# dusk-network/dusk-blindbidproof

Hardware: AMD Instinct MI355X
Metric: blind-bid proofs/sec (higher is better)
Workload: dtype u32

## Files before the change

dusk_blindbidproof_amd/csrc/msm.hip:

```cpp
#include "context.h"

namespace bbp {

#ifndef BBP_FOLD_PRIO
#define BBP_FOLD_PRIO 2
#endif
#ifndef BBP_MSM_WAVES
#define BBP_MSM_WAVES 2
#endif
#ifndef BBP_MSM_WAVES_MAX
#define BBP_MSM_WAVES_MAX 2
#endif

#ifdef BBP_MSM_PROF
__device__ unsigned long long g_msm_prof[8];
#define MSM_PROF_BEGIN() unsigned long long prof_t = wall_clock64()
#define MSM_PROF_MARK(i)                                                    \
    if (tid == 0) {                                                         \
        unsigned long long now_ = wall_clock64();                           \
        atomicAdd(&g_msm_prof[i], now_ - prof_t);                           \
        prof_t = now_;                                                      \
    }
#else
#define MSM_PROF_BEGIN()
#define MSM_PROF_MARK(i)
#endif

__device__ __forceinline__ ge ge_shfl_down(const ge& p, int d) {
    ge r;
    const u32* w = reinterpret_cast<const u32*>(&p);
    u32* o = reinterpret_cast<u32*>(&r);
#pragma unroll
    for (int i = 0; i < GE_WORDS; i++) o[i] = (u32)__shfl_down((int)w[i], d, 64);
    return r;
}

__device__ __forceinline__ void xch_put(u32* xch, const ge& p) {
    const u32* w = reinterpret_cast<const u32*>(&p);
#pragma unroll
    for (int i = 0; i < GE_WORDS; i++) xch[i] = w[i];
}

__device__ __forceinline__ ge xch_get(const u32* xch) {
    ge p;
    u32* w = reinterpret_cast<u32*>(&p);
#pragma unroll
    for (int i = 0; i < GE_WORDS; i++) w[i] = xch[i];
    return p;
}

__device__ __forceinline__ row_regs load_row(const niels_row* __restrict__ tab, u32 entry, u32* __restrict__ fault) {
    u32 row = entry & 0x7fffffffu;
    if (row > (u32)(TAB_BASES * MSM_POS - 1)) {
        row = (u32)(TAB_BASES * MSM_POS - 1);
        atomicOr(fault, 1u);
    }
#ifdef BBP_EXP_ROWMASK
    row &= BBP_EXP_ROWMASK;
#endif
    return load_row_at(tab + row, entry >> 31);
}

#ifdef BBP_ACC_COOP
constexpr int COOP_IMG = 64 * 128;
__device__ __forceinline__ u32 coop_clamp_row(u32 entry, u32* __restrict__ fault) {
    u32 row = entry & 0x7fffffffu;
    if (row > (u32)(TAB_BASES * MSM_POS - 1)) {
        row = (u32)(TAB_BASES * MSM_POS - 1);
        atomicOr(fault, 1u);
    }
    return row;
}
__device__ __forceinline__ void coop_issue(const niels_row* __restrict__ tab, u8* wb, u32 my_row, int lane, u32 srcoff) {
    const u8* t = reinterpret_cast<const u8*>(tab);
    u32 r[8];
#pragma unroll
    for (int j = 0; j < 8; j++) r[j] = (u32)__shfl((int)my_row, 8 * j + (lane >> 3), 64);
#pragma unroll
    for (int j = 0; j < 8; j++) {
        const u8* src = t + (size_t)r[j] * 128 + (srcoff ^ (u32)((j & 1) << 6));
        __builtin_amdgcn_global_load_lds((const __attribute__((address_space(1))) void*)src, (__attribute__((address_space(3))) void*)(wb + j * 1024), 16, 0, 0);
    }
}
__device__ __forceinline__ row_regs coop_read(const u8* wb, u32 A, u32 neg) {
    const u32 An = A ^ (neg << 6);
    const uint4 a0 = *reinterpret_cast<const uint4*>(wb + An), a1 = *reinterpret_cast<const uint4*>(wb + (An ^ 0x10u));
    const uint2 a2 = *reinterpret_cast<const uint2*>(wb + (An ^ 0x20u));
    const uint4 b0 = *reinterpret_cast<const uint4*>(wb + (An ^ 0x40u)), b1 = *reinterpret_cast<const uint4*>(wb + (An ^ 0x50u));
    const uint2 b2 = *reinterpret_cast<const uint2*>(wb + (An ^ 0x60u));
    const uint2 x0 = *reinterpret_cast<const uint2*>(wb + (A ^ 0x20u) + 8);
    const uint4 x1 = *reinterpret_cast<const uint4*>(wb + (A ^ 0x30u));
    const uint2 x2 = *reinterpret_cast<const uint2*>(wb + (A ^ 0x60u) + 8), x3 = *reinterpret_cast<const uint2*>(wb + (A ^ 0x70u));
    row_regs r;
    r.ypx = fe{{(i32)a0.x, (i32)a0.y, (i32)a0.z, (i32)a0.w, (i32)a1.x, (i32)a1.y, (i32)a1.z, (i32)a1.w, (i32)a2.x, (i32)a2.y}};
    r.ymx = fe{{(i32)b0.x, (i32)b0.y, (i32)b0.z, (i32)b0.w, (i32)b1.x, (i32)b1.y, (i32)b1.z, (i32)b1.w, (i32)b2.x, (i32)b2.y}};
    r.xy2d = fe{{(i32)x0.x, (i32)x0.y, (i32)x1.x, (i32)x1.y, (i32)x1.z, (i32)x1.w, (i32)x2.x, (i32)x2.y, (i32)x3.x, (i32)x3.y}};
    return r;
}
#endif

__device__ __noinline__ void ge_add_nc(ge& r, const ge& a, const ge& b) { r = ge_add(a, b); }
__device__ __noinline__ void ge_dbl_nc(ge& r, const ge& a) { r = ge_dbl(a); }

#ifndef BBP_SORT_T
#define BBP_SORT_T 1024
#endif
constexpr int SORT_T = BBP_SORT_T;
template <int MODE> struct msm_geom;
template <> struct msm_geom<0> { static constexpr int K = MSM_K, NAF = MSM_NAF, W = MSM_W; };
template <> struct msm_geom<1> { static constexpr int K = FOLD_K, NAF = FOLD_NAF, W = FOLD_W; };
template <> struct msm_geom<2> { static constexpr int K = SMALL_K, NAF = SMALL_NAF, W = SMALL_W; };

template <int MODE>
__global__ __launch_bounds__(SORT_T) void k_msm_sort(const u32* __restrict__ scal_a, const u32* __restrict__ aux, u32 n_total, u32 n_idx_sets,
                                                      u32 n_sub, u32 split, u32* __restrict__ sorted_all, u32* __restrict__ cursor_all,
                                                      const u32* __restrict__ msm_map, const u32* __restrict__ n_active, u32* __restrict__ ticket) {
    constexpr int K = msm_geom<MODE>::K, NAF = msm_geom<MODE>::NAF, W = msm_geom<MODE>::W, G = K >= SORT_T ? K / SORT_T : 1;
    __shared__ u32 cursor[K + 1];
    __shared__ u32 part[SORT_T];
    const int tid = threadIdx.x;
    if (ticket && blockIdx.x == 0 && tid == 0) *ticket = 0;
    if (n_active && blockIdx.x >= *n_active) return;
    const size_t work = blockIdx.x, msm = work / split;
    const u32 i0 = (u32)(work % split) * n_sub;
    const u32 n = i0 < n_total ? min(n_sub, n_total - i0) : 0u;
    __builtin_amdgcn_s_setprio(3);
    const u32* sbase;
    const u32* base_idx = nullptr;
    u32 base0 = 0;
    if (MODE != 1) {
        const size_t src = msm_map ? (size_t)msm_map[msm] : msm;
        sbase = scal_a + (src * (size_t)n_total + i0) * 8;
        base_idx = aux + (size_t)(msm % n_idx_sets) * n_total + i0;
    } else {
        const u32 side = (u32)msm & 1u;
        sbase = (side ? aux : scal_a) + ((msm >> 1) * (size_t)2048 + i0) * 8;
        base0 = (side ? BBP_BASE_H0 : BBP_BASE_G0) + i0;
    }
    u32* sorted = sorted_all + work * (size_t)n_sub * W;
    auto key = [&](u32 i, u32 mag) -> u32 { return (MODE != 1 ? 0u : ((i0 + i) & (FOLD_CLS - 1)) * FOLD_M) + ((mag + 1) >> 1); };

    for (int k = tid; k <= K; k += SORT_T) cursor[k] = 0;
    __syncthreads();
    for (u32 i = tid; i < n; i += SORT_T) {
        const uint4* sp = reinterpret_cast<const uint4*>(sbase + (size_t)i * 8);
        uint4 lo = sp[0], hi = sp[1];
        const u32 s[8] = {lo.x, lo.y, lo.z, lo.w, hi.x, hi.y, hi.z, hi.w};
        if (MODE != 1 && base_idx[i] == MSM_SKIP_BASE) continue;
        sc_for_each_naf_digit<NAF>(s, [&](u32, u32 mag, u32) { atomicAdd(&cursor[key(i, mag)], 1u); });
    }
    __syncthreads();
    {
        u32 local = 0;
        for (int r = 1; r <= G; r++)
            if (tid * G + r <= K) local += cursor[tid * G + r];
        const int lane = tid & 63, wave = tid >> 6;
        u32 incl = local;
#pragma unroll
        for (int d = 1; d < 64; d <<= 1) {
            const u32 up = (u32)__shfl_up((int)incl, d, 64);
            if (lane >= d) incl += up;
        }
        if (lane == 63) part[wave] = incl;
        __syncthreads();
        if (tid < 64) {
            constexpr int NW = SORT_T / 64;
            u32 v = tid < NW ? part[tid] : 0u, sc_ = v;
#pragma unroll
            for (int d = 1; d < 64; d <<= 1) {
                const u32 up = (u32)__shfl_up((int)sc_, d, 64);
                if (tid >= d) sc_ += up;
            }
            if (tid < NW) part[tid] = sc_ - v;
        }
        __syncthreads();
        u32 base = part[wave] + incl - local;
        for (int r = 1; r <= G; r++) {
            if (tid * G + r > K) break;
            const u32 c = cursor[tid * G + r];
            cursor[tid * G + r] = base;
            base += c;
        }
    }
    __syncthreads();
    for (u32 i = tid; i < n; i += SORT_T) {
        const uint4* sp = reinterpret_cast<const uint4*>(sbase + (size_t)i * 8);
        uint4 lo = sp[0], hi = sp[1];
        const u32 s[8] = {lo.x, lo.y, lo.z, lo.w, hi.x, hi.y, hi.z, hi.w};
        if (MODE != 1 && base_idx[i] == MSM_SKIP_BASE) continue;
        const u32 tb = (MODE != 1 ? base_idx[i] : base0 + i) * MSM_POS;
        sc_for_each_naf_digit<NAF>(s, [&](u32 pos, u32 mag, u32 neg) {
            u32 at = atomicAdd(&cursor[key(i, mag)], 1u);
            sorted[at] = (tb + pos) | (neg << 31);
        });
    }
    __syncthreads();
    u32* cur_out = cursor_all + work * (size_t)(K + 1);
    for (int k = tid; k <= K; k += SORT_T) cur_out[k] = k ? cursor[k] : 0u;
}

template <int MODE> struct sort_cap { static constexpr u32 V = BBP_SORT_CAP; };
#ifndef BBP_SORT_CAP_FOLD
#define BBP_SORT_CAP_FOLD 8192
#endif
template <> struct sort_cap<1> { static constexpr u32 V = BBP_SORT_CAP_FOLD; };
constexpr int SORT_S = 3, SORT_S_WIDE = 5, SORT_S_FOLD = 2;
constexpr int SORT_MAXW = 62;
static_assert((u32)SORT_S_WIDE * SORT_T >= SORT_STAGED_MAX_TERMS && SORT_S_FOLD * SORT_T >= 2048 && SORT_MAXW + 2 <= SORT_T, "staged sort geometry");

#ifdef BBP_MSM_PROF
__device__ unsigned long long g_sort_prof[4][16];
#define SORT_PROF_MARK(i)                                                   \
    if (tid == 0) {                                                         \
        unsigned long long now_ = wall_clock64();                           \
        atomicAdd(&g_sort_prof[prof_cls][(i) < 15 ? (i) : 14], now_ - prof_t); \
        prof_t = now_;                                                      \
    }
#else
#define SORT_PROF_MARK(i)
#endif

template <int MODE, int S>
__global__ __launch_bounds__(SORT_T) void k_msm_sort_staged(const u32* __restrict__ scal_a, const u32* __restrict__ aux, u32 n_total, u32 n_idx_sets,
                                                             u32 n_sub, u32 split, u32* __restrict__ sorted_all, u32* __restrict__ cursor_all,
                                                             const u32* __restrict__ msm_map, const u32* __restrict__ n_active, u32 CAP, u32* __restrict__ ticket) {
    constexpr int K = msm_geom<MODE>::K, NAF = msm_geom<MODE>::NAF, W = msm_geom<MODE>::W, G = K >= SORT_T ? K / SORT_T : 1;
    constexpr int P = naf_slots<NAF>::P, NSLOT = naf_slots<NAF>::N, DW = naf_slots<NAF>::WORDS;
    extern __shared__ u32 stage[];
    __shared__ u32 start[K + 2];
    __shared__ u32 fill[K + 1];
    __shared__ u32 part[SORT_T];
    const int tid = threadIdx.x;
    if (ticket && blockIdx.x == 0 && tid == 0) *ticket = 0;
    if (n_active && blockIdx.x >= *n_active) return;
    const size_t work = blockIdx.x, msm = work / split;
    const u32 i0 = (u32)(work % split) * n_sub;
    const u32 n = i0 < n_total ? min(n_sub, n_total - i0) : 0u;
    __builtin_amdgcn_s_setprio(3);
    const u32* sbase;
    const u32* base_idx = nullptr;
    u32 base0 = 0;
    if (MODE != 1) {
        const size_t src = msm_map ? (size_t)msm_map[msm] : msm;
        sbase = scal_a + (src * (size_t)n_total + i0) * 8;
        base_idx = aux + (size_t)(msm % n_idx_sets) * n_total + i0;
    } else {
        const u32 side = (u32)msm & 1u;
        sbase = (side ? aux : scal_a) + ((msm >> 1) * (size_t)2048 + i0) * 8;
        base0 = (side ? BBP_BASE_H0 : BBP_BASE_G0) + i0;
    }
    u32* sorted = sorted_all + work * (size_t)n_sub * W;
    auto key = [&](u32 i, u32 mag) -> u32 { return (MODE != 1 ? 0u : ((i0 + i) & (FOLD_CLS - 1)) * FOLD_M) + ((mag + 1) >> 1); };

#ifdef BBP_MSM_PROF
    const int prof_cls = MODE == 1 ? 3 : n_sub <= 2049 ? 0 : n_sub <= SORT_WIDE_FROM ? 1 : 2;
    if (tid == 0) atomicAdd(&g_sort_prof[prof_cls][15], 1ull);
    unsigned long long prof_t = wall_clock64();
#endif
    for (int k = tid; k <= K; k += SORT_T) fill[k] = 0;
    __syncthreads();
    u32 dig[S][DW], valid[S], tb[S], koff[S];
#pragma unroll
    for (int j = 0; j < S; j++) {
        const u32 i = (u32)tid + (u32)j * SORT_T;
        valid[j] = 0, tb[j] = 0, koff[j] = 0;
#pragma unroll
        for (int d = 0; d < DW; d++) dig[j][d] = 0;
        if (i < n) {
            const uint4* sp = reinterpret_cast<const uint4*>(sbase + (size_t)i * 8);
            uint4 lo = sp[0], hi = sp[1];
            const u32 s[8] = {lo.x, lo.y, lo.z, lo.w, hi.x, hi.y, hi.z, hi.w};
            const u32 b = MODE != 1 ? base_idx[i] : base0 + i;
            if (MODE == 1 || b != MSM_SKIP_BASE) {
                tb[j] = b * MSM_POS;
                koff[j] = key(i, 0);
                const u32 ko = koff[j];
                sc_naf_digits_packed<NAF>(s, dig[j], valid[j], [&](u32 p) { atomicAdd(&fill[ko + naf_packed_bucket(p)], 1u); });
            }
        }
    }
    __syncthreads();
    SORT_PROF_MARK(0);
    {
        u32 local = 0;
        for (int r = 1; r <= G; r++)
            if (tid * G + r <= K) local += fill[tid * G + r];
        const int lane = tid & 63, wave = tid >> 6;
        u32 incl = local;
#pragma unroll
        for (int d = 1; d < 64; d <<= 1) {
            const u32 up = (u32)__shfl_up((int)incl, d, 64);
            if (lane >= d) incl += up;
        }
        if (lane == 63) part[wave] = incl;
        __syncthreads();
        if (tid < 64) {
            constexpr int NW = SORT_T / 64;
            u32 v = tid < NW ? part[tid] : 0u, sc_ = v;
#pragma unroll
            for (int d = 1; d < 64; d <<= 1) {
                const u32 up = (u32)__shfl_up((int)sc_, d, 64);
                if (tid >= d) sc_ += up;
            }
            if (tid < NW) part[tid] = sc_ - v;
        }
        __syncthreads();
        u32 base = part[wave] + incl - local;
        for (int r = 1; r <= G; r++) {
            if (tid * G + r > K) break;
            const u32 c = fill[tid * G + r];
            start[tid * G + r] = base;
            fill[tid * G + r] = 0;
            base += c;
        }
        if (tid == SORT_T - 1) start[K + 1] = base;
        if (tid == 0) start[0] = 0;
    }
    __syncthreads();
    u32 kb0 = 1;
    while (kb0 <= (u32)K) {
        if (tid < 64) {
            u32 kb = kb0, nw = 0;
            while (kb <= (u32)K && nw < (u32)SORT_MAXW) {
                const u32 base = start[kb];
                u32 ke = kb + 1;
                if (start[ke] - base <= CAP) {
                    u32 lo = kb + 1, hi = (u32)K + 1;
                    while (lo < hi) {
                        const u32 mid = (lo + hi + 1) >> 1;
                        if (start[mid] - base <= CAP) lo = mid; else hi = mid - 1;
                    }
                    ke = lo;
                }
                if (start[ke] != base) {
                    if (tid == 0) part[1 + nw] = ke;
                    nw++;
                }
                kb = ke;
            }
            if (tid == 0) part[0] = nw, part[1 + nw] = kb;
        }
        __syncthreads();
        SORT_PROF_MARK(2);
        const u32 nw = (u32)__builtin_amdgcn_readfirstlane((int)part[0]);
        u32 kb = kb0;
        for (u32 w = 0; w < nw; w++) {
            const u32 ke = (u32)__builtin_amdgcn_readfirstlane((int)part[1 + w]);
            const u32 base = (u32)__builtin_amdgcn_readfirstlane((int)start[kb]), cnt = (u32)__builtin_amdgcn_readfirstlane((int)start[ke]) - base;
            const bool direct = cnt > CAP;
#pragma unroll
            for (int j = 0; j < S; j++) {
                asm volatile("" : "+v"(valid[j]));
#pragma unroll
                for (int d = 0; d < DW; d++) asm volatile("" : "+v"(dig[j][d]));
                if (!valid[j]) continue;
#pragma unroll
                for (int t = 0; t < NSLOT; t++) {
                    if (!(valid[j] >> t & 1)) continue;
                    const u32 p = naf_slot<NAF>(dig[j], t), k = koff[j] + naf_packed_bucket(p);
                    if (k - kb < ke - kb) {
                        const u32 at = start[k] + atomicAdd(&fill[k], 1u);
                        const u32 ent = (tb[j] + naf_packed_pos(p, t / P)) | (naf_packed_neg(p) << 31);
                        if (direct) sorted[at] = ent; else stage[at - base] = ent;
                    }
                }
            }
            __syncthreads();
            SORT_PROF_MARK(3 + 2 * w);
            if (!direct) {
                for (u32 i = tid; i < cnt; i += SORT_T) sorted[base + i] = stage[i];
                __syncthreads();
            }
            SORT_PROF_MARK(4 + 2 * w);
            kb = ke;
        }
        kb0 = (u32)__builtin_amdgcn_readfirstlane((int)part[1 + nw]);
        __syncthreads();
    }
    u32* cur_out = cursor_all + work * (size_t)(K + 1);
    for (int k = tid; k <= K; k += SORT_T) cur_out[k] = k ? start[k + 1] : 0u;
}

#ifndef BBP_ACC_WG
#define BBP_ACC_WG 256
#endif
constexpr int ACC_WG = BBP_ACC_WG, ACC_WGS = ACC_T / ACC_WG;
static_assert(ACC_T % ACC_WG == 0 && ACC_WG % 64 == 0, "accumulate workgroup geometry");

template <int MODE>
__global__ __launch_bounds__(ACC_WG) __attribute__((amdgpu_waves_per_eu(BBP_MSM_WAVES, BBP_MSM_WAVES_MAX)))
void k_msm_acc(const niels_row* __restrict__ ptable, const u32* __restrict__ sorted_all, const u32* __restrict__ cursor_all, u32 n ,
               ge* __restrict__ bsum_all, ge* __restrict__ psum_all, ge* __restrict__ out, const u32* __restrict__ n_active, u32* __restrict__ fault,
               u32 n_work, u32* __restrict__ ticket) {
    constexpr int K = msm_geom<MODE>::K, W = msm_geom<MODE>::W, G = K / MSM_T;
    __shared__ u32 cursor[K + 1];
#ifdef BBP_ACC_PERSIST
    static_assert(ACC_WGS == 1, "the persistent form draws whole MSMs");
    __shared__ u32 s_ticket;
  for (;;) {
    __syncthreads();
    if (threadIdx.x == 0) s_ticket = atomicAdd(ticket, 1u);
    __syncthreads();
    const size_t msm = s_ticket;
    if (msm >= n_work || (n_active && msm >= *n_active)) return;
    const int tid = (int)threadIdx.x;
#else
    const size_t msm = blockIdx.x / ACC_WGS;
    const int tid = (int)(blockIdx.x % ACC_WGS) * ACC_WG + (int)threadIdx.x;
    if (n_active && msm >= *n_active) return;
#endif
    const u32* sorted = sorted_all + msm * (size_t)n * W;
#ifdef BBP_MSM_PRIO
    __builtin_amdgcn_s_setprio(BBP_MSM_PRIO);
#endif
    MSM_PROF_BEGIN();
    {
        const u32* cur_in = cursor_all + msm * (size_t)(K + 1);
        for (int k = threadIdx.x; k <= K; k += ACC_WG) cursor[k] = cur_in[k];
    }
    __syncthreads();
    MSM_PROF_MARK(1);

    const u32 E = cursor[K];
    ge* bsum = bsum_all + msm * (size_t)K;
    ge* psum = psum_all + msm * (size_t)ACC_T;
#ifdef BBP_KO_ACC_PERMILLE
    const u32 c0 = (u32)(((u64)tid * E) / ACC_T), c1 = c0 + (u32)(((u64)((u32)(((u64)(tid + 1) * E) / ACC_T) - c0) * BBP_KO_ACC_PERMILLE) / 1000);
#else
    const u32 c0 = (u32)(((u64)tid * E) / ACC_T), c1 = (u32)(((u64)(tid + 1) * E) / ACC_T);
#endif
#ifdef BBP_MSM_PROF
    const unsigned long long clk0 = clock64();
#endif
    u32 k_first = 0;
    bool inside = false;
#ifdef BBP_ACC_COOP
    {
        __shared__ __attribute__((aligned(1024))) u8 rowimg[ACC_WG / 64][COOP_IMG];
        const int lane = (int)threadIdx.x & 63;
        u8* wb = rowimg[threadIdx.x >> 6];
        const u32 A = (u32)lane * 128u + ((((u32)lane >> 1) & 7u) << 4);
        const u32 srcoff = (((u32)lane & 7u) ^ (((u32)lane >> 3) >> 1)) << 4;
        const u32 n_it = (E + (u32)ACC_T - 1) / (u32)ACC_T, len = c1 - c0;
        u32 k = 1, kend = 0;
        ge* dest = &psum[tid];
        if (len) {
            u32 lo = 1, hi = K;
            while (lo < hi) {
                u32 mid = (lo + hi) >> 1;
                if (cursor[mid] > c0) hi = mid; else lo = mid + 1;
            }
            k = lo, kend = cursor[k];
            k_first = lo;
            inside = cursor[k - 1] < c0;
            if (!inside) dest = &bsum[k - 1];
        }
        ge acc = ge_identity();
        u32 ent_cur = len ? sorted[c0] : 0u;
        u32 ent_nxt = len > 1 ? sorted[c0 + 1] : 0u;
        if (n_it) coop_issue(ptable, wb, coop_clamp_row(ent_cur, fault), lane, srcoff);
        for (u32 it = 0; it < n_it; it++) {
            const u32 e = c0 + it;
            const row_regs cur = coop_read(wb, A, ent_cur >> 31);
            const bool neg = ent_cur >> 31;
            ent_cur = ent_nxt;
            const bool live = it < len;
            if (live && e == kend) {
                *dest = acc;
                acc = ge_identity();
                do { k++; kend = cursor[k]; } while (kend == e);
                dest = &bsum[k - 1];
            }
            asm volatile("s_waitcnt lgkmcnt(0)" ::: "memory");
            if (it + 1 < n_it) coop_issue(ptable, wb, coop_clamp_row(ent_cur, fault), lane, srcoff);
            if (it + 2 < len) ent_nxt = sorted[e + 2]; else ent_nxt = 0u;
            if (live) acc = ge_madd_row(acc, cur, neg);
        }
        if (len) *dest = acc;
    }
#else
    if (c0 < c1) {
        u32 lo = 1, hi = K;
        while (lo < hi) {
            u32 mid = (lo + hi) >> 1;
            if (cursor[mid] > c0) hi = mid; else lo = mid + 1;
        }
        u32 k = lo, kend = cursor[k];
        k_first = lo;
        inside = cursor[k - 1] < c0;
        ge* dest = inside ? &psum[tid] : &bsum[k - 1];
        ge acc = ge_identity();
        u32 ent_cur = sorted[c0];
        u32 ent_nxt = (c0 + 1 < c1) ? sorted[c0 + 1] : 0u;
        row_regs row = load_row(ptable, ent_cur, fault);
        for (u32 e = c0; e < c1; e++) {
            if (e == kend) {
                *dest = acc;
                acc = ge_identity();
                do { k++; kend = cursor[k]; } while (kend == e);
                dest = &bsum[k - 1];
            }
            const row_regs cur = row;
            const bool neg = ent_cur >> 31;
            ent_cur = ent_nxt;
            if (e + 1 < c1) row = load_row(ptable, ent_cur, fault);
            if (e + 2 < c1) ent_nxt = sorted[e + 2];
            acc = ge_madd_row(acc, cur, neg);
        }
        *dest = acc;
    }
#endif
#ifdef BBP_MSM_PROF
    if (tid == 0) atomicAdd(&g_msm_prof[6], clock64() - clk0);
#endif
    MSM_PROF_MARK(2);
    __threadfence_block();
    __syncthreads();
    MSM_PROF_MARK(3);
#ifdef BBP_ACC_PERSIST
  }
#endif
}

template <int MODE>
__global__ __launch_bounds__(MSM_T) void k_msm_fold(const u32* __restrict__ cursor_all, ge* __restrict__ bsum_all, const ge* __restrict__ psum_all,
                                                     ge* __restrict__ out, const u32* __restrict__ n_active) {
    constexpr int K = msm_geom<MODE>::K, G = K / MSM_T;
    __shared__ u32 cursor[K + 1];
    __shared__ u32 xch[GE_WORDS];
    const int tid = threadIdx.x;
    if (n_active && blockIdx.x >= *n_active) return;
    __builtin_amdgcn_s_setprio(BBP_FOLD_PRIO);
    const size_t msm = blockIdx.x;
    {
        const u32* cur_in = cursor_all + msm * (size_t)(K + 1);
        for (int k = tid; k <= K; k += MSM_T) cursor[k] = cur_in[k];
    }
    __syncthreads();
    const u32 E = cursor[K];
    ge* bsum = bsum_all + msm * (size_t)K;
    const ge* psum = psum_all + msm * (size_t)ACC_T;
#ifdef BBP_KO_FOLD
    if (MODE != 1) { if (tid == 0) out[msm] = bsum[0]; }
    else if (tid < FOLD_CLS) out[msm * FOLD_CLS + tid] = bsum[tid];
    return;
#endif
    for (u32 ch = tid; ch < (u32)ACC_T; ch += MSM_T) {
        const u32 c0 = (u32)(((u64)ch * E) / ACC_T), c1 = (u32)(((u64)(ch + 1) * E) / ACC_T);
        if (c0 >= c1) continue;
        u32 lo = 1, hi = K;
        while (lo < hi) {
            u32 mid = (lo + hi) >> 1;
            if (cursor[mid] > c0) hi = mid; else lo = mid + 1;
        }
        const u32 k_first = lo;
        const bool inside = cursor[lo - 1] < c0;
        const bool last_of_run = inside && !(c1 < E && c1 > cursor[k_first - 1] && c1 < cursor[k_first]);
        if (last_of_run) {
            ge part = psum[ch];
            for (int u = (int)ch - 1; u >= 0; u--) {
                const u32 cu = (u32)(((u64)u * E) / ACC_T), cu1 = (u32)(((u64)(u + 1) * E) / ACC_T);
                if (cu <= cursor[k_first - 1]) break;
                if (cu1 > cu) ge_add_nc(part, part, psum[u]);
            }
            ge head = bsum[k_first - 1];
            ge_add_nc(head, head, part);
            bsum[k_first - 1] = head;
        }
    }
    __threadfence_block();
    __syncthreads();

    ge running = ge_identity(), total = ge_identity();
    if constexpr (G == 1) {
        if (cursor[tid + 1] != cursor[tid]) running = bsum[tid];
        total = running;
    } else {
#pragma unroll 1
        for (int r = G; r >= 1; r--) {
            const u32 k = tid * G + r;
            if (cursor[k] != cursor[k - 1]) running = ge_add(running, bsum[k - 1]);
            total = ge_add(total, running);
        }
    }

    if constexpr (MODE != 1) {
        const int lane = tid & 63, wave = tid >> 6;
#pragma unroll 1
        for (int d = 1; d < 64; d <<= 1) {
            ge other = ge_shfl_down(running, d);
            if (lane + d < 64) running = ge_add(running, other);
        }
        if (MSM_T > 64) {
            if (tid == 64) xch_put(xch, running);
            __syncthreads();
            if (wave == 0) {
                ge other = xch_get(xch);
                ge_add_nc(running, running, other);
            }
        }
        ge x = total;
        if (tid >= 1) {
            ge s = running;
            constexpr int LOG_G = G == 1 ? 0 : G == 2 ? 1 : G == 4 ? 2 : G == 8 ? 3 : G == 16 ? 4 : -1;
            static_assert(LOG_G >= 0, "buckets per fold lane must be a power of two up to 16");
            for (int i = 0; i < LOG_G; i++) ge_dbl_nc(s, s);
            ge_add_nc(x, x, s);
        }
#pragma unroll 1
        for (int d = 32; d >= 1; d >>= 1) {
            ge other = ge_shfl_down(x, d);
            if (lane < d) x = ge_add(x, other);
        }
        if (MSM_T > 64) {
            __syncthreads();
            if (tid == 64) xch_put(xch, x);
            __syncthreads();
        }
        if (tid == 0) {
            if (MSM_T > 64) {
                ge other = xch_get(xch);
                ge_add_nc(x, x, other);
            }
            ge other;
            ge_dbl_nc(x, x);
            other = ge_neg(running);
            ge_add_nc(x, x, other);
            out[msm] = x;
        }
    } else {
        constexpr int LPC = FOLD_M / G, LOG_G2 = G == 32 ? 5 : 6;
        static_assert(G == 32 || G == 64, "class reduction written for 4 or 2 lanes per class");
        const int q = tid & (LPC - 1);
        ge suf = running;
        for (int d = 1; d < LPC; d++) {
            ge other = ge_shfl_down(running, d);
            if (q + d < LPC) ge_add_nc(suf, suf, other);
        }
        ge x = total;
        if (q >= 1) {
            ge sg = suf;
            for (int i = 0; i < LOG_G2; i++) ge_dbl_nc(sg, sg);
            ge_add_nc(x, x, sg);
        }
        ge accq = x;
        for (int d = 1; d < LPC; d++) {
            ge other = ge_shfl_down(x, d);
            if (q == 0) ge_add_nc(accq, accq, other);
        }
        if (q == 0) {
            ge_dbl_nc(accq, accq);
            ge other = ge_neg(suf);
            ge_add_nc(accq, accq, other);
            out[msm * FOLD_CLS + (tid / LPC)] = accq;
        }
    }
}

constexpr int FOLD2_L = 32;
constexpr int FOLD2_G = MSM_K / FOLD2_L;
constexpr int FOLD2_LOG_G = 5;
static_assert(FOLD2_G == 32 && ACC_T % FOLD2_L == 0, "fold geometry");

__device__ __forceinline__ ge ge_shfl_down32(const ge& p, int d) {
    ge r;
    const u32* w = reinterpret_cast<const u32*>(&p);
    u32* o = reinterpret_cast<u32*>(&r);
#pragma unroll
    for (int i = 0; i < GE_WORDS; i++) o[i] = (u32)__shfl_down((int)w[i], d, 32);
    return r;
}

__device__ __forceinline__ ge ge_add_t2d(const ge& p, const fe& p2d, const ge& q) {
    fe a = fe_mul(fe_sub(p.Y, p.X), fe_sub(q.Y, q.X));
    fe b = fe_mul(fe_add(p.Y, p.X), fe_add(q.Y, q.X));
    fe c = fe_mul(p2d, q.T);
    fe zz = fe_mul(p.Z, q.Z);
    fe d = fe_add(zz, zz);
    fe e = fe_sub(b, a), f = fe_sub(d, c), g = fe_add(d, c), h = fe_add(b, a);
    ge r;
    r.X = fe_mul(e, f);
    r.Y = fe_mul(g, h);
    r.Z = fe_mul(g, f);
    r.T = fe_mul(e, h);
    return r;
}

__device__ __forceinline__ void park_put(u32* park, int tid, const ge& p) {
    const u32* w = reinterpret_cast<const u32*>(&p);
#pragma unroll
    for (int i = 0; i < GE_WORDS; i++) park[i * 64 + tid] = w[i];
}

__device__ __forceinline__ ge park_get(const u32* park, int tid) {
    ge p;
    u32* w = reinterpret_cast<u32*>(&p);
#pragma unroll
    for (int i = 0; i < GE_WORDS; i++) w[i] = park[i * 64 + tid];
    return p;
}

__device__ __forceinline__ ge ld_ge(const ge* p) {
    ge r;
    const uint4* s = reinterpret_cast<const uint4*>(p);
    u32* o = reinterpret_cast<u32*>(&r);
#pragma unroll
    for (int i = 0; i < GE_WORDS / 4; i++) {
        const uint4 v = s[i];
        o[4 * i] = v.x, o[4 * i + 1] = v.y, o[4 * i + 2] = v.z, o[4 * i + 3] = v.w;
    }
    return r;
}

#ifndef BBP_FOLD_WAVES
#define BBP_FOLD_WAVES 2
#endif
__global__ __launch_bounds__(64) __attribute__((amdgpu_waves_per_eu(BBP_FOLD_WAVES, BBP_FOLD_WAVES))) void k_msm_fold_half(const u32* __restrict__ cursor_all, ge* __restrict__ bsum_all, const ge* __restrict__ psum_all,
                                                       ge* __restrict__ out, u32 n_work, const u32* __restrict__ n_active) {
    constexpr int K = MSM_K, G = FOLD2_G;
    __shared__ u32 cursor2[2][K + 1];
    __shared__ u32 park[GE_WORDS * 64];
    const int tid = threadIdx.x, half = tid >> 5, l = tid & 31;
    const u32 n_tot = n_active ? min(*n_active, n_work) : n_work;
    if (2u * blockIdx.x >= n_tot) return;
    __builtin_amdgcn_s_setprio(BBP_FOLD_PRIO);
    const size_t msm = 2 * (size_t)blockIdx.x + half;
    const bool valid = msm < n_tot;
    u32* cursor = cursor2[half];
    {
        const u32* cur_in = cursor_all + msm * (size_t)(K + 1);
        for (int k = l; k <= K; k += FOLD2_L) cursor[k] = valid ? cur_in[k] : 0u;
    }
    __syncthreads();
    const u32 E = cursor[K];
    ge* bsum = bsum_all + (valid ? msm : 0) * (size_t)K;
    const ge* psum = psum_all + (valid ? msm : 0) * (size_t)ACC_T;
#pragma unroll 1
    for (u32 ch = l; ch < (u32)ACC_T; ch += FOLD2_L) {
        const u32 c0 = (u32)(((u64)ch * E) / ACC_T), c1 = (u32)(((u64)(ch + 1) * E) / ACC_T);
        bool last_of_run = false;
        u32 k_first = 1;
        if (c0 < c1) {
            u32 lo = 1, hi = K;
            while (lo < hi) {
                u32 mid = (lo + hi) >> 1;
                if (cursor[mid] > c0) hi = mid; else lo = mid + 1;
            }
            k_first = lo;
            const bool inside = cursor[lo - 1] < c0;
            last_of_run = inside && !(c1 < E && c1 > cursor[k_first - 1] && c1 < cursor[k_first]);
        }
        if (last_of_run) {
            ge part = ld_ge(&psum[ch]);
            for (int u = (int)ch - 1; u >= 0; u--) {
                const u32 cu = (u32)(((u64)u * E) / ACC_T), cu1 = (u32)(((u64)(u + 1) * E) / ACC_T);
                if (cu <= cursor[k_first - 1]) break;
                if (cu1 > cu) {
                    const ge more = ld_ge(&psum[u]);
                    part = ge_add(part, more);
                }
            }
            const ge head = ld_ge(&bsum[k_first - 1]);
            bsum[k_first - 1] = ge_add(head, part);
        }
    }
    __threadfence_block();
    __syncthreads();

    ge running = ge_identity();
    fe r2d = fe_zero();
    park_put(park, tid, ge_identity());
#pragma unroll 1
    for (int r = G; r >= 1; r--) {
        const u32 k = (u32)l * G + r;
        if (cursor[k] != cursor[k - 1]) {
            const ge cur = ld_ge(&bsum[k - 1]);
            running = ge_add_t2d(running, r2d, cur);
            r2d = fe_mul(running.T, fe_d2());
        }
        const ge total = park_get(park, tid);
        park_put(park, tid, ge_add_t2d(running, r2d, total));
    }

    ge v = running;
#pragma unroll 1
    for (int it = 0; it < 12; it++) {
        ge q;
        bool take;
        int n_dbl = 0;
        if (it == 5) {
            q = v;
            v = park_get(park, tid);
            park_put(park, tid, q);
            n_dbl = FOLD2_LOG_G;
            take = l >= 1;
        } else if (it == 11) {
            q = ge_neg(park_get(park, tid));
            take = true;
        } else {
            const int d = it < 5 ? (1 << it) : (16 >> (it - 6));
            q = ge_shfl_down32(v, d);
            take = it < 5 ? (l + d < 32) : (l < d);
        }
        if (it == 11) {
            v = ge_dbl(v);
        } else {
#pragma unroll 1
            for (int i = 0; i < n_dbl; i++) q = ge_dbl(q);
        }
        if (take) v = ge_add(v, q);
    }
    if (l == 0 && valid) out[msm] = v;
}

constexpr int REDUCE_L = 16;
__global__ __launch_bounds__(64) void k_msm_reduce(u32 n_out, u32 split, u32 items, const ge* __restrict__ tmp, ge* __restrict__ out) {
    __builtin_amdgcn_s_setprio(3);
    const u32 t = blockIdx.x * blockDim.x + threadIdx.x;
    const u32 o = t / REDUCE_L, j = t % REDUCE_L;
    const u32 msm = o / items, c = o % items;
    ge acc = ge_identity();
    if (o < n_out && j < split) acc = tmp[((size_t)msm * split + j) * items + c];
    for (u32 jj = j + REDUCE_L; o < n_out && jj < split; jj += REDUCE_L)
        acc = ge_add(acc, tmp[((size_t)msm * split + jj) * items + c]);
#pragma unroll 1
    for (int d = REDUCE_L / 2; d >= 1; d >>= 1) {
        const ge other = ge_shfl_down(acc, d);
        if ((int)j < d) acc = ge_add(acc, other);
    }
    if (o < n_out && j == 0) out[o] = acc;
}


struct MsmScratch {
    u32 *sorted, *cursor;
    ge *bsum, *psum, *tmp;
    u32* ticket;
    size_t bytes;
};
static MsmScratch msm_scratch_layout(void* base, size_t n_msm, size_t n_terms, size_t W, size_t K, size_t out_items = 1) {
    auto up = [](size_t x) { return (x + 255) / 256 * 256; };
    MsmScratch m;
    size_t o = 0;
    m.sorted = reinterpret_cast<u32*>(static_cast<u8*>(base) + o);
    o += up(n_msm * n_terms * W * sizeof(u32));
    m.cursor = reinterpret_cast<u32*>(static_cast<u8*>(base) + o);
    o += up(n_msm * (K + 1) * sizeof(u32));
    m.bsum = reinterpret_cast<ge*>(static_cast<u8*>(base) + o);
    o += n_msm * K * sizeof(ge);
    m.psum = reinterpret_cast<ge*>(static_cast<u8*>(base) + o);
    o += n_msm * ACC_T * sizeof(ge);
    m.tmp = reinterpret_cast<ge*>(static_cast<u8*>(base) + o);
    o += up(n_msm * out_items * sizeof(ge));
    m.ticket = reinterpret_cast<u32*>(static_cast<u8*>(base) + o);
    o += 256;
    m.bytes = o;
    return m;
}
size_t msm_scratch_bytes(uint32_t n_msm, uint32_t n_terms) {
    const u32 split = msm_split(n_msm, n_terms), n_sub = (n_terms + split - 1) / split;
    size_t a = msm_scratch_layout(nullptr, (size_t)n_msm * split, n_sub, MSM_W, MSM_K).bytes;
    if (split > 1) a = std::max(a, msm_scratch_layout(nullptr, (size_t)n_msm * split, n_sub, SMALL_W, SMALL_K).bytes);
    const size_t b = msm_scratch_layout(nullptr, n_msm, n_terms, MSM_W, MSM_K).bytes;
    return a > b ? a : b;
}

static inline u32 acc_grid(bbp_ctx*, u32 n_work) {
#ifdef BBP_ACC_PERSIST
    static const u32 cap = [] { const char* e = getenv("BBP_ACC_PERSIST_GRID"); return e ? (u32)atoi(e) : 512u; }();
    return n_work < cap ? n_work : cap;
#else
    return n_work * ACC_WGS;
#endif
}

int32_t fold_generators_launch(bbp_ctx* ctx, uint32_t n_proofs, const sc* g_dev, const sc* h_dev, ge* out_dev, hipStream_t stream,
                               int scratch_slot) {
    if (n_proofs == 0) return BBP_OK;
    const size_t n_msm = 2 * (size_t)n_proofs;
    const u32 split = msm_split((u32)n_msm, 2048), n_sub = (2048 + split - 1) / split;
    const size_t n_work = n_msm * split;
    DevBuf& scratch = ctx->slice_fold[scratch_slot];
    int32_t rc = dev_reserve(ctx, scratch, msm_scratch_layout(nullptr, n_work, n_sub, FOLD_W, FOLD_K, FOLD_CLS).bytes);
    if (rc) return rc;
    const MsmScratch m = msm_scratch_layout(scratch.p, n_work, n_sub, FOLD_W, FOLD_K, FOLD_CLS);
    {
        ScopedEvent ev(ctx, TAG_MSM_SORT, stream);
        if (ctx->msm_knobs.sort_staged & 2) {
            if (!ctx->sort_lds_attr1) {
                BBP_HIP_TRY(ctx, hipFuncSetAttribute((const void*)k_msm_sort_staged<1, SORT_S_FOLD>, hipFuncAttributeMaxDynamicSharedMemorySize, (int)(sort_cap<1>::V * 4)));
                ctx->sort_lds_attr1 = true;
            }
            hipLaunchKernelGGL((k_msm_sort_staged<1, SORT_S_FOLD>), dim3((u32)n_work), dim3(SORT_T), sort_cap<1>::V * 4, stream, (const u32*)g_dev, (const u32*)h_dev, 2048u, 1u,
                               n_sub, split, m.sorted, m.cursor, (const u32*)nullptr, (const u32*)nullptr, sort_cap<1>::V, m.ticket);
        } else
            hipLaunchKernelGGL(k_msm_sort<1>, dim3((u32)n_work), dim3(SORT_T), 0, stream, (const u32*)g_dev, (const u32*)h_dev, 2048u, 1u, n_sub, split,
                               m.sorted, m.cursor, (const u32*)nullptr, (const u32*)nullptr, m.ticket);
        BBP_HIP_TRY(ctx, hipGetLastError());
    }
    {
        ScopedEvent ev(ctx, TAG_MSM, stream);
        hipLaunchKernelGGL(k_msm_acc<1>, dim3(acc_grid(ctx, (u32)n_work)), dim3(ACC_WG), 0, stream, ctx->ptable, m.sorted, m.cursor, n_sub, m.bsum, m.psum,
                           split > 1 ? m.tmp : out_dev, (const u32*)nullptr, ctx->health, (u32)n_work, m.ticket);
        BBP_HIP_TRY(ctx, hipGetLastError());
    }
    ScopedEvent evf(ctx, TAG_MSM_FOLD, stream);
    hipLaunchKernelGGL(k_msm_fold<1>, dim3((u32)n_work), dim3(MSM_T), 0, stream, m.cursor, m.bsum, m.psum, split > 1 ? m.tmp : out_dev,
                       (const u32*)nullptr);
    BBP_HIP_TRY(ctx, hipGetLastError());
    if (split > 1) {
        const u32 n_out = (u32)n_msm * FOLD_CLS;
        hipLaunchKernelGGL(k_msm_reduce, dim3((n_out * REDUCE_L + 63) / 64), dim3(64), lds_token(ctx), stream, n_out, split, (u32)FOLD_CLS, m.tmp, out_dev);
        BBP_HIP_TRY(ctx, hipGetLastError());
    }
    return BBP_OK;
}

__global__ __launch_bounds__(64) void k_encode(const ge* __restrict__ pts, u32 n, u32* __restrict__ out_words) {
    u32 i = blockIdx.x * blockDim.x + threadIdx.x;
    if (i >= n) return;
    ge p = pts[i];
    u32 w[8];
    ge_encode_words(w, p);
    uint4* o = reinterpret_cast<uint4*>(out_words + (size_t)i * 8);
    o[0] = make_uint4(w[0], w[1], w[2], w[3]);
    o[1] = make_uint4(w[4], w[5], w[6], w[7]);
}

__global__ void k_debug_poke(u32* sorted) { sorted[0] = 0x7ffffff0u; }

int32_t msm_launch(bbp_ctx* ctx, uint32_t n_msm, uint32_t n_terms, const u32* scalars_dev, const u32* base_idx_dev,
                   ge* out_points_dev, hipStream_t stream, uint32_t n_idx_sets, int scratch_slot, const u32* msm_map_dev,
                   const u32* n_active_dev, bool chain_acc) {
    if (n_msm == 0) return BBP_OK;
    if (n_terms == 0 || n_terms > 65535u) {
        ctx->err = "msm_launch: n_terms out of range";
        return BBP_ERR_BAD_ARG;
    }
    DevBuf& scratch = scratch_slot ? ctx->slice_sorted[scratch_slot] : ctx->sorted;
    int32_t rc = dev_reserve(ctx, scratch, msm_scratch_bytes(n_msm, n_terms));
    if (rc) return rc;
    const MsmPlan plan = plan_msm(ctx->msm_knobs, n_msm, n_terms, n_active_dev != nullptr);
    const u32 split = plan.split, n_sub = plan.n_sub, n_work = plan.n_work;
    if (plan.geom == MsmPlan::SMALL) {
        const MsmScratch ms = msm_scratch_layout(scratch.p, n_work, n_sub, SMALL_W, SMALL_K);
        {
            ScopedEvent ev(ctx, TAG_MSM_SORT, stream);
            hipLaunchKernelGGL(k_msm_sort<2>, dim3(n_work), dim3(SORT_T), 0, stream, scalars_dev, base_idx_dev, n_terms, n_idx_sets, n_sub, split, ms.sorted, ms.cursor,
                               msm_map_dev, n_active_dev, ms.ticket);
            BBP_HIP_TRY(ctx, hipGetLastError());
        }
        if (ctx->debug_corrupt) {
            ctx->debug_corrupt = 0;
            hipLaunchKernelGGL(k_debug_poke, dim3(1), dim3(1), 0, stream, ms.sorted);
            BBP_HIP_TRY(ctx, hipGetLastError());
        }
        {
            ScopedEvent ev(ctx, TAG_MSM, stream);
            hipLaunchKernelGGL(k_msm_acc<2>, dim3(acc_grid(ctx, n_work)), dim3(ACC_WG), 0, stream, ctx->ptable, ms.sorted, ms.cursor, n_sub, ms.bsum, ms.psum, ms.tmp,
                               n_active_dev, ctx->health, n_work, ms.ticket);
            BBP_HIP_TRY(ctx, hipGetLastError());
        }
        {
            ScopedEvent evf(ctx, TAG_MSM_FOLD, stream);
            hipLaunchKernelGGL(k_msm_fold<2>, dim3(n_work), dim3(MSM_T), 0, stream, ms.cursor, ms.bsum, ms.psum, ms.tmp, n_active_dev);
            BBP_HIP_TRY(ctx, hipGetLastError());
        }
        hipLaunchKernelGGL(k_msm_reduce, dim3((n_msm * REDUCE_L + 63) / 64), dim3(64), lds_token(ctx), stream, n_msm, split, 1u, ms.tmp, out_points_dev);
        BBP_HIP_TRY(ctx, hipGetLastError());
        return BBP_OK;
    }
    const MsmScratch m = msm_scratch_layout(scratch.p, n_work, n_sub, MSM_W, MSM_K);
    {
        ScopedEvent ev(ctx, TAG_MSM_SORT, stream);
        if (plan.sort != MsmPlan::PLAIN) {
            const u32 cap = plan.sort_cap;
            if (!ctx->sort_lds_attr) {
                BBP_HIP_TRY(ctx, hipFuncSetAttribute((const void*)k_msm_sort_staged<0, SORT_S>, hipFuncAttributeMaxDynamicSharedMemorySize, (int)(SORT_CAP_WIDE * 4)));
                BBP_HIP_TRY(ctx, hipFuncSetAttribute((const void*)k_msm_sort_staged<0, SORT_S_WIDE>, hipFuncAttributeMaxDynamicSharedMemorySize, (int)(SORT_CAP_WIDE * 4)));
                ctx->sort_lds_attr = true;
            }
            if (n_sub > (u32)SORT_S_WIDE * SORT_T) {
                ctx->err = "msm_launch: staged sort planned for more terms than its lanes hold";
                return BBP_ERR_INTERNAL;
            }
            if (n_sub <= (u32)SORT_S * SORT_T)
                hipLaunchKernelGGL((k_msm_sort_staged<0, SORT_S>), dim3(n_work), dim3(SORT_T), cap * 4, stream, scalars_dev, base_idx_dev, n_terms, n_idx_sets, n_sub, split,
                                   m.sorted, m.cursor, msm_map_dev, n_active_dev, cap, m.ticket);
            else
                hipLaunchKernelGGL((k_msm_sort_staged<0, SORT_S_WIDE>), dim3(n_work), dim3(SORT_T), cap * 4, stream, scalars_dev, base_idx_dev, n_terms, n_idx_sets, n_sub, split,
                                   m.sorted, m.cursor, msm_map_dev, n_active_dev, cap, m.ticket);
        }
        else
            hipLaunchKernelGGL(k_msm_sort<0>, dim3(n_work), dim3(SORT_T), 0, stream, scalars_dev, base_idx_dev, n_terms, n_idx_sets, n_sub, split,
                               m.sorted, m.cursor, msm_map_dev, n_active_dev, m.ticket);
        BBP_HIP_TRY(ctx, hipGetLastError());
    }
    if (ctx->debug_corrupt) {
        ctx->debug_corrupt = 0;
        hipLaunchKernelGGL(k_debug_poke, dim3(1), dim3(1), 0, stream, m.sorted);
        BBP_HIP_TRY(ctx, hipGetLastError());
    }
    chain_acc = chain_acc && ctx->verify_serial_acc;
    if (chain_acc && ctx->vacc_valid)
        BBP_HIP_TRY(ctx, hipStreamWaitEvent(stream, ctx->ev_vacc[ctx->vacc_seq % bbp_ctx::VACC_RING], 0));
    {
        ScopedEvent ev(ctx, TAG_MSM, stream);
        hipLaunchKernelGGL(k_msm_acc<0>, dim3(acc_grid(ctx, n_work)), dim3(ACC_WG), 0, stream, ctx->ptable, m.sorted, m.cursor, n_sub, m.bsum, m.psum,
                           split > 1 ? m.tmp : out_points_dev, n_active_dev, ctx->health, n_work, m.ticket);
        BBP_HIP_TRY(ctx, hipGetLastError());
    }
    static const bool chain_after_fold = getenv("BBP_VERIFY_CHAIN_AFTER_FOLD") && atoi(getenv("BBP_VERIFY_CHAIN_AFTER_FOLD"));
    if (chain_acc && !chain_after_fold) {
        ctx->vacc_seq++;
        BBP_HIP_TRY(ctx, hipEventRecord(ctx->ev_vacc[ctx->vacc_seq % bbp_ctx::VACC_RING], stream));
        ctx->vacc_valid = true;
    }
    ScopedEvent evf(ctx, TAG_MSM_FOLD, stream);
    if (plan.fold == MsmPlan::HALF)
        hipLaunchKernelGGL(k_msm_fold_half, dim3((n_work + 1) / 2), dim3(64), 0, stream, m.cursor, m.bsum, m.psum, split > 1 ? m.tmp : out_points_dev,
                           n_work, n_active_dev);
    else
        hipLaunchKernelGGL(k_msm_fold<0>, dim3(n_work), dim3(MSM_T), 0, stream, m.cursor, m.bsum, m.psum, split > 1 ? m.tmp : out_points_dev, n_active_dev);
    BBP_HIP_TRY(ctx, hipGetLastError());
    if (chain_acc && chain_after_fold) {
        ctx->vacc_seq++;
        BBP_HIP_TRY(ctx, hipEventRecord(ctx->ev_vacc[ctx->vacc_seq % bbp_ctx::VACC_RING], stream));
        ctx->vacc_valid = true;
    }
    if (plan.reduce) {
        hipLaunchKernelGGL(k_msm_reduce, dim3((n_msm * REDUCE_L + 63) / 64), dim3(64), lds_token(ctx), stream, n_msm, split, 1u, m.tmp, out_points_dev);
        BBP_HIP_TRY(ctx, hipGetLastError());
    }
#ifdef BBP_MSM_PROF
    static int launches = 0;
    if (++launches % 16 == 0) {
        unsigned long long h[8], sp[4][16];
        (void)hipStreamSynchronize(stream);
        (void)hipMemcpyFromSymbol(sp, HIP_SYMBOL(g_sort_prof), sizeof sp);
        for (int c = 0; c < 4; c++) {
            if (!sp[c][15]) continue;
            fprintf(stderr, "[sort prof class %d, %llu workgroups, 10ns ticks of lane 0 per workgroup]", c, sp[c][15]);
            for (int i = 0; i < 15; i++) fprintf(stderr, " %.1f", (double)sp[c][i] / (double)sp[c][15]);
            fprintf(stderr, "\n");
        }
        (void)hipMemcpyFromSymbol(h, HIP_SYMBOL(g_msm_prof), sizeof h);
        fprintf(stderr, "[msm prof, %d launches, 10ns ticks of lane 0 summed over WGs] load %llu D1 %llu D1wait %llu D2 %llu E %llu; D1 shader clock %.0f MHz\n", launches,
                h[1], h[2], h[3], h[4], h[5], 100.0 * (double)h[6] / (double)h[2]);
    }
#endif
    return BBP_OK;
}

int32_t encode_launch(bbp_ctx* ctx, uint32_t n, const ge* pts_dev, uint8_t* out32_dev, hipStream_t stream) {
    if (n == 0) return BBP_OK;
    ScopedEvent ev(ctx, TAG_ENCODE, stream);
    hipLaunchKernelGGL(k_encode, dim3((n + 63) / 64), dim3(64), lds_token(ctx), stream, pts_dev, n, (u32*)out32_dev);
    BBP_HIP_TRY(ctx, hipGetLastError());
    return BBP_OK;
}

}
```

Measured before the change: 22020.

## Stream fold bucket sums through LDS with async global_load_lds and strided ownership

Reworks k_msm_fold_half so each lane owns buckets strided by FOLD2_L instead of a contiguous block of G buckets. Each step's bucket-sum slice is fetched with global_load_lds DMA into a shared staging image, double-issued ahead of the add chain, so the point loads overlap with the extended-coordinate adds and are coalesced across lanes. It also rewrites the run-tail psum accumulation to fold directly into the bucket value, loads the cursors with a register prefetch, and adjusts the final park/shuffle combine to match the new bucket order. The changes add manual waitcnt ordering and reuse the cursor LDS for staging, which is fragile. It also adds profiling and knockout instrumentation behind macros.

Result: no change. 22240, median of 3 (+1.0%).

```diff
diff --git a/dusk_blindbidproof_amd/csrc/msm.hip b/dusk_blindbidproof_amd/csrc/msm.hip
--- a/dusk_blindbidproof_amd/csrc/msm.hip
+++ b/dusk_blindbidproof_amd/csrc/msm.hip
@@ -4,6 +4,9 @@
 
 #ifndef BBP_FOLD_PRIO
 #define BBP_FOLD_PRIO 2
+#endif
+#ifndef BBP_FOLD_LAYOUT
+#define BBP_FOLD_LAYOUT 1
 #endif
 #ifndef BBP_MSM_WAVES
 #define BBP_MSM_WAVES 2
@@ -21,9 +24,17 @@
         atomicAdd(&g_msm_prof[i], now_ - prof_t);                           \
         prof_t = now_;                                                      \
     }
+__device__ unsigned long long g_fold_prof[5];
+#define FOLD_PROF_MARK(i)                                                   \
+    if (tid == 0) {                                                         \
+        unsigned long long now_ = wall_clock64();                           \
+        atomicAdd(&g_fold_prof[i], now_ - prof_t);                          \
+        prof_t = now_;                                                      \
+    }
 #else
 #define MSM_PROF_BEGIN()
 #define MSM_PROF_MARK(i)
+#define FOLD_PROF_MARK(i)
 #endif
 
 __device__ __forceinline__ ge ge_shfl_down(const ge& p, int d) {
@@ -101,6 +112,7 @@
 
 __device__ __noinline__ void ge_add_nc(ge& r, const ge& a, const ge& b) { r = ge_add(a, b); }
 __device__ __noinline__ void ge_dbl_nc(ge& r, const ge& a) { r = ge_dbl(a); }
+
 
 #ifndef BBP_SORT_T
 #define BBP_SORT_T 1024
@@ -579,7 +591,11 @@
 #pragma unroll 1
         for (int r = G; r >= 1; r--) {
             const u32 k = tid * G + r;
+#ifdef BBP_KO_FOLD_NOLOAD
+            if (cursor[k] != cursor[k - 1]) running = ge_add(running, ge{running.Y, running.X, running.T, running.Z});
+#else
             if (cursor[k] != cursor[k - 1]) running = ge_add(running, bsum[k - 1]);
+#endif
             total = ge_add(total, running);
         }
     }
@@ -712,25 +728,70 @@
     return r;
 }
 
+#if BBP_FOLD_LAYOUT
+constexpr int FOLD2_SPAN = FOLD2_L * (int)sizeof(ge);
+constexpr int FOLD2_DMA = 2 * FOLD2_SPAN / 1024;
+static_assert(sizeof(ge) == GE_WORDS * 4 && sizeof(ge) % 16 == 0 && FOLD2_SPAN % 512 == 0 && FOLD2_DMA * 1024 == GE_WORDS * 64 * 4, "fold step image");
+__device__ __forceinline__ void fold_issue(const u8* src_lane, u8* img) {
+#pragma unroll
+    for (int i = 0; i < FOLD2_DMA; i++)
+        __builtin_amdgcn_global_load_lds((const __attribute__((address_space(1))) void*)(src_lane + i * 512), (__attribute__((address_space(3))) void*)(img + i * 1024), 16, 0, 0);
+}
+__device__ __forceinline__ ge fold_read(const u8* img, int half, int l) {
+    ge r;
+    u32* o = reinterpret_cast<u32*>(&r);
+#pragma unroll
+    for (int i = 0; i < GE_WORDS / 4; i++) {
+        const u32 at = (u32)l * (u32)sizeof(ge) + 16u * i;
+        const uint4 v = *reinterpret_cast<const uint4*>(img + ((at >> 9) << 10) + ((u32)half << 9) + (at & 511u));
+        o[4 * i] = v.x, o[4 * i + 1] = v.y, o[4 * i + 2] = v.z, o[4 * i + 3] = v.w;
+    }
+    return r;
+}
+#endif
+
 #ifndef BBP_FOLD_WAVES
 #define BBP_FOLD_WAVES 2
 #endif
 __global__ __launch_bounds__(64) __attribute__((amdgpu_waves_per_eu(BBP_FOLD_WAVES, BBP_FOLD_WAVES))) void k_msm_fold_half(const u32* __restrict__ cursor_all, ge* __restrict__ bsum_all, const ge* __restrict__ psum_all,
                                                        ge* __restrict__ out, u32 n_work, const u32* __restrict__ n_active) {
     constexpr int K = MSM_K, G = FOLD2_G;
+#if BBP_FOLD_LAYOUT
+    __shared__ __attribute__((aligned(1024))) u32 stage[GE_WORDS * 64];
+    static_assert(2 * (K + 1) <= GE_WORDS * 64, "the two cursors fit in the step image");
+    u32(*cursor2)[K + 1] = reinterpret_cast<u32(*)[K + 1]>(stage);
+#else
     __shared__ u32 cursor2[2][K + 1];
+#endif
     __shared__ u32 park[GE_WORDS * 64];
     const int tid = threadIdx.x, half = tid >> 5, l = tid & 31;
     const u32 n_tot = n_active ? min(*n_active, n_work) : n_work;
     if (2u * blockIdx.x >= n_tot) return;
     __builtin_amdgcn_s_setprio(BBP_FOLD_PRIO);
+    MSM_PROF_BEGIN();
+#ifdef BBP_MSM_PROF
+    const unsigned long long prof_t0 = prof_t;
+#endif
     const size_t msm = 2 * (size_t)blockIdx.x + half;
     const bool valid = msm < n_tot;
     u32* cursor = cursor2[half];
+#if BBP_FOLD_LAYOUT
+    {
+        const u32* cur_in = cursor_all + (valid ? msm : 0) * (size_t)(K + 1);
+        constexpr int NC = K / FOLD2_L + 1;
+        u32 cv[NC];
+#pragma unroll
+        for (int j = 0; j < NC; j++) cv[j] = cur_in[min(l + j * FOLD2_L, K)];
+#pragma unroll
+        for (int j = 0; j < NC; j++)
+            if (l + j * FOLD2_L <= K) cursor[l + j * FOLD2_L] = valid ? cv[j] : 0u;
+    }
+#else
     {
         const u32* cur_in = cursor_all + msm * (size_t)(K + 1);
         for (int k = l; k <= K; k += FOLD2_L) cursor[k] = valid ? cur_in[k] : 0u;
     }
+#endif
     __syncthreads();
     const u32 E = cursor[K];
     ge* bsum = bsum_all + (valid ? msm : 0) * (size_t)K;
@@ -750,6 +811,27 @@
             const bool inside = cursor[lo - 1] < c0;
             last_of_run = inside && !(c1 < E && c1 > cursor[k_first - 1] && c1 < cursor[k_first]);
         }
+#if BBP_FOLD_LAYOUT
+        if (last_of_run) {
+            ge acc = ld_ge(&bsum[k_first - 1]);
+            ge more = ld_ge(&psum[ch]);
+            int u = (int)ch - 1;
+            for (;;) {
+                acc = ge_add(acc, more);
+                bool again = false;
+                for (; u >= 0 && !again; u--) {
+                    const u32 cu = (u32)(((u64)u * E) / ACC_T), cu1 = (u32)(((u64)(u + 1) * E) / ACC_T);
+                    if (cu <= cursor[k_first - 1]) { u = 0; continue; }
+                    if (cu1 > cu) {
+                        more = ld_ge(&psum[u]);
+                        again = true;
+                    }
+                }
+                if (!again) break;
+            }
+            bsum[k_first - 1] = acc;
+        }
+#else
         if (last_of_run) {
             ge part = ld_ge(&psum[ch]);
             for (int u = (int)ch - 1; u >= 0; u--) {
@@ -763,24 +845,67 @@
             const ge head = ld_ge(&bsum[k_first - 1]);
             bsum[k_first - 1] = ge_add(head, part);
         }
+#endif
     }
     __threadfence_block();
     __syncthreads();
+    FOLD_PROF_MARK(0);
 
     ge running = ge_identity();
     fe r2d = fe_zero();
     park_put(park, tid, ge_identity());
+#ifdef BBP_KO_FOLD_NOLOAD
+#define FOLD_KO_CUR(cur) ge cur; cur.X = running.Y, cur.Y = running.X, cur.Z = running.T, cur.T = running.Z
+#endif
+#if BBP_FOLD_LAYOUT
+    u32 nonempty = 0;
+    for (int r = 0; r < G; r++) {
+        const u32 k = (u32)r * FOLD2_L + l + 1;
+        nonempty |= (u32)(cursor[k] != cursor[k - 1]) << r;
+    }
+    __syncthreads();
+    u8* img = reinterpret_cast<u8*>(stage);
+    const u8* src_lane = reinterpret_cast<const u8*>(bsum) + l * 16;
+#ifndef BBP_KO_FOLD_NOLOAD
+    fold_issue(src_lane + (G - 1) * FOLD2_SPAN, img);
+#endif
+#pragma unroll 1
+    for (int r = G - 1; r >= 0; r--) {
+#ifdef BBP_KO_FOLD_NOLOAD
+        FOLD_KO_CUR(cur);
+#else
+        asm volatile("s_waitcnt vmcnt(0)" ::: "memory");
+        const ge cur = fold_read(img, half, l);
+        asm volatile("s_waitcnt lgkmcnt(0)" ::: "memory");
+        if (r > 0) fold_issue(src_lane + (r - 1) * FOLD2_SPAN, img);
+#endif
+        if ((nonempty >> r) & 1u) {
+            running = ge_add_t2d(running, r2d, cur);
+            r2d = fe_mul(running.T, fe_d2());
+        }
+        if (r > 0) {
+            const ge total = park_get(park, tid);
+            park_put(park, tid, ge_add_t2d(running, r2d, total));
+        }
+    }
+#else
 #pragma unroll 1
     for (int r = G; r >= 1; r--) {
         const u32 k = (u32)l * G + r;
         if (cursor[k] != cursor[k - 1]) {
+#ifdef BBP_KO_FOLD_NOLOAD
+            FOLD_KO_CUR(cur);
+#else
             const ge cur = ld_ge(&bsum[k - 1]);
+#endif
             running = ge_add_t2d(running, r2d, cur);
             r2d = fe_mul(running.T, fe_d2());
         }
         const ge total = park_get(park, tid);
         park_put(park, tid, ge_add_t2d(running, r2d, total));
     }
+#endif
+    FOLD_PROF_MARK(1);
 
     ge v = running;
 #pragma unroll 1
@@ -789,11 +914,18 @@
         bool take;
         int n_dbl = 0;
         if (it == 5) {
+#if BBP_FOLD_LAYOUT
+            q = park_get(park, tid);
+            park_put(park, tid, v);
+            n_dbl = FOLD2_LOG_G;
+            take = true;
+#else
             q = v;
             v = park_get(park, tid);
             park_put(park, tid, q);
             n_dbl = FOLD2_LOG_G;
             take = l >= 1;
+#endif
         } else if (it == 11) {
             q = ge_neg(park_get(park, tid));
             take = true;
@@ -811,6 +943,13 @@
         if (take) v = ge_add(v, q);
     }
     if (l == 0 && valid) out[msm] = v;
+    FOLD_PROF_MARK(2);
+#ifdef BBP_MSM_PROF
+    if (tid == 0) {
+        atomicAdd(&g_fold_prof[3], 1ull);
+        atomicMax(&g_fold_prof[4], prof_t - prof_t0);
+    }
+#endif
 }
 
 constexpr int REDUCE_L = 16;
@@ -1044,6 +1183,11 @@
             for (int i = 0; i < 15; i++) fprintf(stderr, " %.1f", (double)sp[c][i] / (double)sp[c][15]);
             fprintf(stderr, "\n");
         }
+        unsigned long long fp[5];
+        (void)hipMemcpyFromSymbol(fp, HIP_SYMBOL(g_fold_prof), sizeof fp);
+        if (fp[3])
+            fprintf(stderr, "[fold_half prof, %llu workgroups, 10ns ticks of lane 0 per workgroup] P %.1f D2 %.1f E %.1f, slowest workgroup %llu\n", fp[3], (double)fp[0] / (double)fp[3],
+                    (double)fp[1] / (double)fp[3], (double)fp[2] / (double)fp[3], fp[4]);
         (void)hipMemcpyFromSymbol(h, HIP_SYMBOL(g_msm_prof), sizeof h);
         fprintf(stderr, "[msm prof, %d launches, 10ns ticks of lane 0 summed over WGs] load %llu D1 %llu D1wait %llu D2 %llu E %llu; D1 shader clock %.0f MHz\n", launches,
                 h[1], h[2], h[3], h[4], h[5], 100.0 * (double)h[6] / (double)h[2]);
```
